# ppwwyyxx/speaker-recognition

Measured on AMD Instinct MI355X. Metric: frames/sec scored (MFCC+GMM), higher is better.
Workload: dtype f32

## Files before the change

### speaker-recognition_amd/csrc/mfcc_f64.hip

```cpp
#include "batch.hpp"
#include "mfcc.hpp"
#include "mfcc_dev.hpp"
#include "wave_ops.hpp"

#include <algorithm>

namespace sr {

static int &precision_flag() {
    static int v = 2;
    return v;
}
int mfcc_precision() { return precision_flag(); }
void mfcc_set_precision(int mode) { precision_flag() = mode == 0 ? 0 : 2; }

using d2 = double2;

__device__ __forceinline__ d2 mk(double x, double y) { return make_double2(x, y); }
__device__ __forceinline__ d2 dadd(d2 a, d2 b) { return mk(a.x + b.x, a.y + b.y); }
__device__ __forceinline__ d2 dsub(d2 a, d2 b) { return mk(a.x - b.x, a.y - b.y); }
__device__ __forceinline__ d2 dmul(d2 a, d2 b) { return mk(fma(-a.y, b.y, a.x * b.x), fma(a.y, b.x, a.x * b.y)); }
__device__ __forceinline__ d2 dmul_mi(d2 a) { return mk(a.y, -a.x); }
constexpr double DH = 0.70710678118654752440;
__device__ __forceinline__ d2 dmul_h_mh(d2 a) { return mk(DH * (a.x + a.y), DH * (a.y - a.x)); }
__device__ __forceinline__ d2 dmul_mh_mh(d2 a) { return mk(DH * (a.y - a.x), -DH * (a.x + a.y)); }

__device__ __forceinline__ d2 tw64(const d2 *t, int i, int nc) {
    d2 w = t[i & (nc - 1)];
    if (i & nc) w = mk(-w.x, -w.y);
    return w;
}

__device__ __forceinline__ void radix4d(d2 a, d2 b, d2 c, d2 d, d2 &y0, d2 &y1, d2 &y2, d2 &y3) {
    const d2 s0 = dadd(a, c), s1 = dsub(a, c), s2 = dadd(b, d), s3 = dmul_mi(dsub(b, d));
    y0 = dadd(s0, s2);
    y1 = dadd(s1, s3);
    y2 = dsub(s0, s2);
    y3 = dsub(s1, s3);
}

template <int NZ>
__device__ __forceinline__ void dft16d(d2 (&v)[16]) {
    constexpr double C1 = 0.92387953251128673848, S1 = 0.38268343236508978178;
    d2 u[4][4];
    if constexpr (NZ <= 4) {
#pragma unroll
        for (int q = 0; q < 4; q++)
#pragma unroll
            for (int r = 0; r < 4; r++) u[q][r] = v[q];
    } else {
#pragma unroll
        for (int q = 0; q < 4; q++) radix4d(v[q], v[4 + q], v[8 + q], v[12 + q], u[q][0], u[q][1], u[q][2], u[q][3]);
    }
    u[1][1] = dmul(u[1][1], mk(C1, -S1));
    u[1][2] = dmul_h_mh(u[1][2]);
    u[1][3] = dmul(u[1][3], mk(S1, -C1));
    u[2][1] = dmul_h_mh(u[2][1]);
    u[2][2] = dmul_mi(u[2][2]);
    u[2][3] = dmul_mh_mh(u[2][3]);
    u[3][1] = dmul(u[3][1], mk(S1, -C1));
    u[3][2] = dmul_mh_mh(u[3][2]);
    u[3][3] = dmul(u[3][3], mk(-C1, S1));
#pragma unroll
    for (int r = 0; r < 4; r++) radix4d(u[0][r], u[1][r], u[2][r], u[3][r], v[r], v[r + 4], v[r + 8], v[r + 12]);
}

template <int CTRL>
__device__ __forceinline__ float quad_f32(float x) {
    return __int_as_float(__builtin_amdgcn_update_dpp(0, __float_as_int(x), CTRL, 0xf, 0xf, true));
}
template <int CTRL>
__device__ __forceinline__ double quad_f64(double x) {
    union { double d; int i[2]; } a, b;
    a.d = x;
    b.i[0] = __builtin_amdgcn_update_dpp(0, a.i[0], CTRL, 0xf, 0xf, true);
    b.i[1] = __builtin_amdgcn_update_dpp(0, a.i[1], CTRL, 0xf, 0xf, true);
    return b.d;
}
constexpr int QUAD_XOR1 = 0xB1;
constexpr int QUAD_XOR2 = 0x4E;

__device__ constexpr double W32_COS[9] = {1.0, 0.98078528040323044913, 0.92387953251128675613, 0.83146961230254523708,
                                          0.70710678118654752440, 0.55557023301960222474, 0.38268343236508977173,
                                          0.19509032201612826785, 0.0};

__device__ __forceinline__ double ln_pos_f32(float e) {
    int ex;
    float m = frexpf(e, &ex);
    if (m < 0.70710678f) {
        m *= 2.0f;
        ex -= 1;
    }
    const double md = (double)m, den = md + 1.0;
    double r = (double)__builtin_amdgcn_rcpf((float)den);
    r = fma(r, fma(-den, r, 1.0), r);
    const double s = (md - 1.0) * r, s2 = s * s;
    double c15 = 1.0 / 15.0, c13 = 1.0 / 13.0, c11 = 1.0 / 11.0, c9 = 1.0 / 9.0, c7 = 1.0 / 7.0, c5 = 1.0 / 5.0, c3 = 1.0 / 3.0, ln2 = 0.69314718055994530942;
    asm volatile("" : "+s"(c15), "+s"(c13), "+s"(c11), "+s"(c9), "+s"(c7), "+s"(c5), "+s"(c3), "+s"(ln2));
    double p = c15;
    p = fma(p, s2, c13);
    p = fma(p, s2, c11);
    p = fma(p, s2, c9);
    p = fma(p, s2, c7);
    p = fma(p, s2, c5);
    p = fma(p, s2, c3);
    p = fma(p, s2, 1.0);
    return fma((double)ex, ln2, 2.0 * s * p);
}

constexpr int F64_WIN_BYTES = 4160;
constexpr int F64_WPB = 8;
constexpr int F64_U_ELEMS = 576;
constexpr int F64_PBUF_BYTE = F64_U_ELEMS * 16;
constexpr int F64_SE_BYTE = F64_PBUF_BYTE + 1100 * 4;
constexpr int F64_SLM_BYTE = F64_SE_BYTE + 272;
static_assert(F64_SLM_BYTE % 32 == 0 && F64_SLM_BYTE + 512 <= WAVE_SLAB_C * 16, "per-wave slab layout");

template <typename PcmT, int MP>
__global__ __launch_bounds__(64 * F64_WPB)
void mfcc_frames_fft2048_f64_kernel(const PcmT *__restrict__ pcm, const int64_t *__restrict__ sample_off,
                                    const int64_t *__restrict__ frame_off, int n_utt, int64_t n_frames,
                                    int64_t frames_per_wave, MfccDev p, MfccDev64 q, MelRuns mr, float *__restrict__ raw) {
    extern __shared__ __attribute__((aligned(32))) char smem[];
    constexpr int NC = 1024;
    float *s_melval = reinterpret_cast<float *>(smem);
    const int lane = threadIdx.x & 63;
    const int wave = threadIdx.x >> 6;
    double *s_win = reinterpret_cast<double *>(smem + (((size_t)mr.pad_floats * 4 + 31) & ~(size_t)31));
    char *slab_b = reinterpret_cast<char *>(s_win) + F64_WIN_BYTES + (size_t)wave * WAVE_SLAB_C * sizeof(d2);
    d2 *slab = reinterpret_cast<d2 *>(slab_b);
    float *pbuf = reinterpret_cast<float *>(slab_b + F64_PBUF_BYTE);
    float *s_e = reinterpret_cast<float *>(slab_b + F64_SE_BYTE);
    double *s_lm = reinterpret_cast<double *>(slab_b + F64_SLM_BYTE);

    for (int i = threadIdx.x; i < mr.pad_floats; i += 64 * F64_WPB) s_melval[i] = mr.pad_val[i];
    for (int i = threadIdx.x; i < F64_WIN_BYTES / 8; i += 64 * F64_WPB) s_win[i] = (i >= 1 && i <= p.frame_len) ? q.window[i - 1] : 0.0;
    __syncthreads();

    const d2 w1 = q.twiddle[2 * lane];
    const d2 wl = q.twiddle[lane];
    const int bb = lane & 15, gg = lane >> 4;
    const d2 w64_1 = q.twiddle[32 * bb];
    const int L = p.frame_len;
    const double lm_floor = q.mel_floor[lane];
    const int m_part = lane & 3, m_bl = lane >> 2;
    int m_c0[4];
#pragma unroll
    for (int ps = 0; ps < 4; ps++) m_c0[ps] = mr.col0[16 * ps + m_bl];

    const int64_t gwave = (int64_t)blockIdx.x * F64_WPB + wave;
    const int64_t f_begin = gwave * frames_per_wave;
    const int64_t f_end = f_begin + frames_per_wave < n_frames ? f_begin + frames_per_wave : n_frames;
    if (f_begin >= f_end) return;

    int utt = 0;
    {
        int lo = 0, hi = n_utt;
        while (hi - lo > 1) {
            const int mid = (lo + hi) >> 1;
            if (frame_off[mid] <= f_begin) lo = mid; else hi = mid;
        }
        utt = lo;
    }
    int64_t utt_f0 = frame_off[utt], utt_f1 = frame_off[utt + 1], utt_s0 = sample_off[utt];

    PcmT cm[4], c0[4], c1[4];
    auto fetch = [&](int64_t base) {
        const PcmT *fp = pcm + base;
#pragma unroll
        for (int n1 = 0; n1 < 4; n1++) {
            const int i0 = 2 * (64 * n1 + lane);
            c0[n1] = fp[min(i0, L - 1)];
            cm[n1] = fp[max(min(i0 - 1, L - 1), 0)];
            c1[n1] = fp[min(i0 + 1, L - 1)];
        }
    };
    fetch(utt_s0 + (f_begin - utt_f0) * p.frame_shift);

    for (int64_t frame = f_begin; frame < f_end; frame++) {
        d2 v[16];
#pragma unroll
        for (int n1 = 0; n1 < 4; n1++) {
            const int i0 = 2 * (64 * n1 + lane);
            const d2 wm0 = *reinterpret_cast<const d2 *>(s_win + i0);
            const double wp1 = s_win[i0 + 2];
            const double x0 = (double)c0[n1], xm = (double)cm[n1], x1 = (double)c1[n1];
            const double y0 = wm0.y * x0;
            const double re = fma(-(wm0.x * q.pre_emph), xm, y0);
            const double im = fma(-q.pre_emph, y0, wp1 * x1);
            v[n1] = mk(i0 < L ? re : 0.0, i0 + 1 < L ? im : 0.0);
        }
        if (frame + 1 < f_end) {
            int64_t nf = frame + 1;
            while (nf >= utt_f1) {
                utt++;
                utt_f0 = utt_f1;
                utt_f1 = frame_off[utt + 1];
                utt_s0 = sample_off[utt];
            }
            fetch(utt_s0 + (nf - utt_f0) * p.frame_shift);
        }
        dft16d<4>(v);
        {
            d2 cur = w1;
            v[1] = dmul(v[1], cur);
#pragma unroll
            for (int k1 = 2; k1 < 16; k1++) {
                cur = dmul(cur, w1);
                v[k1] = dmul(v[k1], cur);
            }
        }
        wave_sync();
#pragma unroll
        for (int k1 = 0; k1 < 16; k1++) slab[k1 * 68 + lane] = v[k1];
        wave_sync();
        {
            d2 w64_2 = dmul(w64_1, w64_1);
            asm volatile("" : "+v"(w64_2.x), "+v"(w64_2.y));
            const d2 w64_3 = dmul(w64_2, w64_1);
#pragma unroll
            for (int i = 0; i < 4; i++) {
                const d2 *rowp = slab + (4 * gg + i) * 68 + bb;
                radix4d(rowp[0], rowp[16], rowp[32], rowp[48], v[4 * i], v[4 * i + 1], v[4 * i + 2], v[4 * i + 3]);
                v[4 * i + 1] = dmul(v[4 * i + 1], w64_1);
                v[4 * i + 2] = dmul(v[4 * i + 2], w64_2);
                v[4 * i + 3] = dmul(v[4 * i + 3], w64_3);
            }
        }
        wave_sync();
#pragma unroll
        for (int i = 0; i < 4; i++)
#pragma unroll
            for (int c = 0; c < 4; c++) slab[((4 * gg + i) + 16 * c) * 17 + bb] = v[4 * i + c];
        wave_sync();
#pragma unroll
        for (int b = 0; b < 16; b++) v[b] = slab[lane * 17 + b];
        dft16d<16>(v);
        wave_sync();
#pragma unroll
        for (int d = 8; d < 16; d++) slab[(d - 8) * 64 + lane] = v[d];
        wave_sync();
        {
            const int src = (64 - lane) & 63;
            const int shift = lane == 0 ? 64 : 0;
#pragma unroll
            for (int d = 0; d < 8; d++) {
                const d2 zk = v[d];
                d2 zr = slab[(7 - d) * 64 + shift + src];
                if (d == 0 && lane == 0) zr = zk;
                const d2 e = mk(zk.x + zr.x, zk.y - zr.y);
                const d2 o = mk(zk.y + zr.y, zr.x - zk.x);
                d2 t;
                if (d == 0) t = dmul(wl, o);
                else if (d == 4) t = dmul(wl, dmul_h_mh(o));
                else t = dmul(wl, dmul(mk(W32_COS[d], -W32_COS[8 - d]), o));
                const d2 xp = dadd(e, t), xm = dsub(e, t);
                const int k = lane + 64 * d;
                pbuf[k] = (float)fma(xp.x, xp.x, xp.y * xp.y);
                pbuf[NC - k] = (float)fma(xm.x, xm.x, xm.y * xm.y);
            }
            if (lane == 0) pbuf[512] = (float)(4.0 * fma(v[8].x, v[8].x, v[8].y * v[8].y));
            pbuf[1025 + lane] = 0.f;
            if (lane < 11) pbuf[1089 + lane] = 0.f;
        }
        double dw[4][4];
        int dct_lane = lane;
        asm volatile("" : "+v"(dct_lane));
#pragma unroll
        for (int it = 0; it < 4; it++) {
            const double4 wv = reinterpret_cast<const double4 *>(q.dct_pad)[it * 64 + dct_lane];
            dw[it][0] = wv.x; dw[it][1] = wv.y; dw[it][2] = wv.z; dw[it][3] = wv.w;
        }
        wave_sync();
#pragma unroll
        for (int ps = 0; ps < 4; ps++) {
            const int len = mr.pass_len[ps];
            const float4 *mv4 = reinterpret_cast<const float4 *>(s_melval + mr.pass_base[ps]) + lane;
            int c0v = m_c0[ps];
            if constexpr (MP == 0) {
                int bl = 16 * ps + m_bl;
                asm volatile("" : "+v"(bl));
                c0v = mr.col0[bl];
            }
            const float4 *pp4 = reinterpret_cast<const float4 *>(pbuf + c0v) + m_part;
            float a0 = 0.f, a1 = 0.f, a2 = 0.f, a3 = 0.f;
            if constexpr (MP != 0) {
#pragma unroll
                for (int it = 0; it < mel_preset_steps(MP, ps); it++) {
                    const float4 wv = mv4[it * 64];
                    const float4 xv = pp4[it * 4];
                    a0 = fmaf(wv.x, xv.x, a0);
                    a1 = fmaf(wv.y, xv.y, a1);
                    a2 = fmaf(wv.z, xv.z, a2);
                    a3 = fmaf(wv.w, xv.w, a3);
                }
            } else {
                for (int it = 0; it < (len >> 4); it++) {
                    const float4 wv = mv4[it * 64];
                    const float4 xv = pp4[it * 4];
                    a0 = fmaf(wv.x, xv.x, a0);
                    a1 = fmaf(wv.y, xv.y, a1);
                    a2 = fmaf(wv.z, xv.z, a2);
                    a3 = fmaf(wv.w, xv.w, a3);
                }
            }
            float acc = (a0 + a1) + (a2 + a3);
            acc += quad_f32<QUAD_XOR1>(acc);
            acc += quad_f32<QUAD_XOR2>(acc);
            if (m_part == 0) s_e[16 * ps + m_bl] = acc;
        }
        wave_sync();
        {
            const float e = s_e[lane];
            s_lm[lane] = e > 0.f ? ln_pos_f32(e) : lm_floor;
        }
        wave_sync();
        {
            const int cidx = lane >> 2;
            const double4 *lp = reinterpret_cast<const double4 *>(s_lm) + m_part;
            double o0 = 0.0, o1 = 0.0;
#pragma unroll
            for (int it = 0; it < 4; it++) {
                const double4 lv = lp[it * 4];
                o0 = fma(dw[it][0], lv.x, o0);
                o1 = fma(dw[it][1], lv.y, o1);
                o0 = fma(dw[it][2], lv.z, o0);
                o1 = fma(dw[it][3], lv.w, o1);
            }
            double o = o0 + o1;
            o += quad_f64<QUAD_XOR1>(o);
            o += quad_f64<QUAD_XOR2>(o);
            if (m_part == 0 && cidx < p.n_ceps) raw[frame * p.n_ceps + cidx] = (float)o;
        }
    }
}

template <typename PcmT, int WPB>
__global__ __launch_bounds__(64 * WPB)
void mfcc_frames_f64_kernel(const PcmT *__restrict__ pcm, const int64_t *__restrict__ sample_off,
                            const int64_t *__restrict__ frame_off, int n_utt, int64_t n_frames,
                            MfccDev p, MfccDev64 q, float *__restrict__ raw ) {
    extern __shared__ __attribute__((aligned(16))) char smem[];
    const int nc = p.fft_size >> 1;
    d2 *s_tw = reinterpret_cast<d2 *>(smem);
    const int lane = threadIdx.x & 63;
    const int wave = threadIdx.x >> 6;
    d2 *buf_a = s_tw + nc + (size_t)wave * 2 * nc;
    d2 *buf_b = buf_a + nc;
    double *s_lm = reinterpret_cast<double *>(s_tw + nc + (size_t)WPB * 2 * nc) + wave * 64;

    for (int i = threadIdx.x; i < nc; i += 64 * WPB) s_tw[i] = q.twiddle[i];
    __syncthreads();

    const int64_t frames_per_iter = (int64_t)gridDim.x * WPB;
    const int64_t iters = (n_frames + frames_per_iter - 1) / frames_per_iter;
    for (int64_t it = 0; it < iters; it++) {
        const int64_t frame = (it * gridDim.x + blockIdx.x) * WPB + wave;
        const bool active = frame < n_frames;

        int64_t base = 0;
        if (active) {
            int lo = 0, hi = n_utt;
            while (hi - lo > 1) {
                const int mid = (lo + hi) >> 1;
                if (frame_off[mid] <= frame) lo = mid; else hi = mid;
            }
            base = sample_off[lo] + (frame - frame_off[lo]) * p.frame_shift;
        }

        if (active) {
            const int L = p.frame_len;
            for (int n = lane; n < nc; n += 64) {
                double re = 0.0, im = 0.0;
                const int i0 = 2 * n;
                if (i0 < L) {
                    const double c0 = (double)pcm[base + i0] * q.window[i0];
                    const double pm1 = i0 > 0 ? (double)pcm[base + i0 - 1] * q.window[i0 - 1] : 0.0;
                    re = i0 > 0 ? c0 - pm1 * q.pre_emph : c0;
                    if (i0 + 1 < L) {
                        const double c1 = (double)pcm[base + i0 + 1] * q.window[i0 + 1];
                        im = c1 - c0 * q.pre_emph;
                    }
                }
                buf_a[n] = mk(re, im);
            }
        }
        __syncthreads();

        d2 *in = buf_a, *out = buf_b;
        int ns = 1;
        for (; ns * 4 <= nc; ns *= 4) {
            if (active) {
                const int T = nc >> 2;
                const int tstep = p.fft_size / (4 * ns);
                for (int j = lane; j < T; j += 64) {
                    const int k = j & (ns - 1);
                    const int qq = k * tstep;
                    const d2 v0 = in[j];
                    const d2 v1 = dmul(in[j + T], tw64(s_tw, qq, nc));
                    const d2 v2 = dmul(in[j + 2 * T], tw64(s_tw, 2 * qq, nc));
                    const d2 v3 = dmul(in[j + 3 * T], tw64(s_tw, 3 * qq, nc));
                    d2 y0, y1, y2, y3;
                    radix4d(v0, v1, v2, v3, y0, y1, y2, y3);
                    const int j0 = ((j - k) << 2) + k;
                    out[j0] = y0;
                    out[j0 + ns] = y1;
                    out[j0 + 2 * ns] = y2;
                    out[j0 + 3 * ns] = y3;
                }
            }
            __syncthreads();
            d2 *t = in; in = out; out = t;
        }
        if (ns < nc) {
            if (active) {
                const int T = nc >> 1;
                for (int j = lane; j < T; j += 64) {
                    const d2 v0 = in[j];
                    const d2 v1 = dmul(in[j + T], tw64(s_tw, 2 * j, nc));
                    out[j] = dadd(v0, v1);
                    out[j + T] = dsub(v0, v1);
                }
            }
            __syncthreads();
            d2 *t = in; in = out; out = t;
        }

        double *pw = reinterpret_cast<double *>(out);
        if (active) {
            for (int k = lane; k <= nc; k += 64) {
                const d2 zk = in[k & (nc - 1)];
                const d2 zr = in[(nc - k) & (nc - 1)];
                const d2 e = mk(0.5 * (zk.x + zr.x), 0.5 * (zk.y - zr.y));
                const d2 o = mk(0.5 * (zk.y + zr.y), -0.5 * (zk.x - zr.x));
                const d2 x = dadd(e, dmul(tw64(s_tw, k, nc), o));
                const double pk = fma(x.x, x.x, x.y * x.y);
                pw[k] = pk < 1e-100 ? 1e-100 : pk;
            }
        }
        __syncthreads();

        if (active) {
            double mine = 0.0;
            for (int b = 0; b < p.n_filters; b++) {
                double acc = 0.0;
                const int e1 = p.mel_row[b + 1];
                for (int e = p.mel_row[b] + lane; e < e1; e += 64) acc = fma(q.mel_val[e], pw[p.mel_col[e]], acc);
                acc = wave_sum_f64(acc);
                if (lane == b) mine = acc > 0.0 ? log(acc) : q.mel_floor[b];
            }
            s_lm[lane] = mine;
        }
        __syncthreads();

        if (active && lane < p.n_ceps) {
            double acc = 0.0;
            const double *drow = q.dct + lane * p.n_filters;
            for (int b = 0; b < p.n_filters; b++) acc = fma(drow[b], s_lm[b], acc);
            raw[frame * p.n_ceps + lane] = (float)acc;
        }
        __syncthreads();
    }
}

void mfcc_launch_f64(SRMfcc &m, const MfccDev &dev, int pcm_kind, const void *pcm, const int64_t *d_pcm_off, const int64_t *d_raw_off,
                     int n_utt, int64_t n_frames, float *raw) {
    auto &tabs = device_tables(m);
    const MfccDev64 dev64 = device_tables_f64(m);
    const size_t mel_bytes = ((size_t)tabs.pad_floats * 4 + 31) & ~(size_t)31;
    const size_t lds_fast = mel_bytes + F64_WIN_BYTES + (size_t)F64_WPB * WAVE_SLAB_C * sizeof(d2);
    const bool fast = m.fft_size == 2048 && m.frame_len <= 512 && tabs.runs_contiguous && m.n_ceps <= 16 &&
                      lds_fast <= (size_t)160 * 1024 && !mfcc_force_generic();
    if (fast) {
        MelRuns mr;
        mr.col0 = tabs.mel_col0.p;
        mr.pad_val = tabs.mel_pad.p;
        mr.pad_floats = tabs.pad_floats;
        for (int ps = 0; ps < 4; ps++) {
            mr.pass_base[ps] = tabs.pass_base[ps];
            mr.pass_len[ps] = tabs.pass_len[ps];
        }
        const int64_t one_round = (int64_t)ctx().n_cu * F64_WPB;
        int64_t frames_per_wave = 1, best_cost = -1;
        for (int64_t r = 1; r <= 4; r++) {
            const int64_t fpw = std::max<int64_t>(1, (n_frames + r * one_round - 1) / (r * one_round));
            const int64_t waves = (n_frames + fpw - 1) / fpw;
            const int64_t cost = ((waves + one_round - 1) / one_round) * fpw;
            if (best_cost < 0 || cost < best_cost - best_cost / 50 || (cost <= best_cost + best_cost / 50 && fpw >= 32)) {
                best_cost = cost;
                frames_per_wave = fpw;
            }
        }
        const int64_t n_waves = (n_frames + frames_per_wave - 1) / frames_per_wave;
        const int grid = (int)((n_waves + F64_WPB - 1) / F64_WPB);
        int preset = 0;
        for (int pr = 1; pr <= 2 && !preset; pr++) {
            bool same = true;
            for (int ps = 0; ps < 4; ps++) same = same && tabs.pass_len[ps] == 16 * mel_preset_steps(pr, ps);
            if (same) preset = pr;
        }
#define SR_LAUNCH_F64(PT, MPV)                                                                              \
    do {                                                                                                     \
        auto kern = mfcc_frames_fft2048_f64_kernel<PT, MPV>;                                                 \
        SR_HIP(hipFuncSetAttribute(reinterpret_cast<const void *>(kern), hipFuncAttributeMaxDynamicSharedMemorySize, (int)lds_fast)); \
        hipLaunchKernelGGL(kern, dim3(grid), dim3(64 * F64_WPB), lds_fast, ctx().stream, static_cast<const PT *>(pcm), d_pcm_off,      \
                           d_raw_off, n_utt, n_frames, frames_per_wave, dev, dev64, mr, raw);                \
    } while (0)
#define SR_LAUNCH_F64_P(PT)                                                                                 \
    do {                                                                                                     \
        if (preset == 1) SR_LAUNCH_F64(PT, 1); else if (preset == 2) SR_LAUNCH_F64(PT, 2); else SR_LAUNCH_F64(PT, 0); \
    } while (0)
        if (pcm_kind == SRBatch::PCM16) SR_LAUNCH_F64_P(int16_t); else SR_LAUNCH_F64_P(float);
#undef SR_LAUNCH_F64_P
#undef SR_LAUNCH_F64
        return;
    }
    const int nc = m.fft_size / 2;
    auto lds_for = [&](int w) { return (size_t)nc * sizeof(d2) * (1 + 2 * w) + (size_t)w * 64 * sizeof(double); };
    const int wpb = lds_for(4) <= (size_t)160 * 1024 ? 4 : lds_for(2) <= (size_t)160 * 1024 ? 2 : 1;
    const size_t lds = lds_for(wpb);
    const int64_t blocks_needed = (n_frames + wpb - 1) / wpb;
    const int blocks_per_cu = std::max<int>(1, (int)(160 * 1024 / lds));
    const int grid = (int)std::min<int64_t>(blocks_needed, (int64_t)ctx().n_cu * std::min(blocks_per_cu, 8));
#define SR_LAUNCH_G64(PT, W)                                                                                \
    do {                                                                                                     \
        auto kern = mfcc_frames_f64_kernel<PT, W>;                                                           \
        SR_HIP(hipFuncSetAttribute(reinterpret_cast<const void *>(kern), hipFuncAttributeMaxDynamicSharedMemorySize, (int)lds)); \
        hipLaunchKernelGGL(kern, dim3(grid), dim3(64 * W), lds, ctx().stream, static_cast<const PT *>(pcm), d_pcm_off, d_raw_off, \
                           n_utt, n_frames, dev, dev64, raw);                                                \
    } while (0)
#define SR_LAUNCH_G64_W(PT)                                                                                 \
    do {                                                                                                     \
        if (wpb == 4) SR_LAUNCH_G64(PT, 4); else if (wpb == 2) SR_LAUNCH_G64(PT, 2); else SR_LAUNCH_G64(PT, 1); \
    } while (0)
    if (pcm_kind == SRBatch::PCM16) SR_LAUNCH_G64_W(int16_t); else SR_LAUNCH_G64_W(float);
#undef SR_LAUNCH_G64_W
#undef SR_LAUNCH_G64
}

}
```

Baseline: 37.11 million.

## Split each f64 MFCC frame across a two-wave team instead of one wave

The fp64 fast-path kernel now processes each frame with a 128-thread team of two waves, each doing half of the 1024-point complex FFT (radix-4 first stage with per-half twiddles, then two radix-8 stages). The untangle step and the mel filterbank sweep are divided between the two waves, and the DCT is left to wave 0. The mel weights are now read from global memory into registers instead of from an LDS copy, which shrinks LDS per block and allows more resident teams per CU. The aim is to cut per-wave register pressure and serial work per frame and raise occupancy, at the cost of block-level barriers and the DCT running on only one wave.

```diff
diff --git a/speaker-recognition_amd/csrc/mfcc_f64.hip b/speaker-recognition_amd/csrc/mfcc_f64.hip
--- a/speaker-recognition_amd/csrc/mfcc_f64.hip
+++ b/speaker-recognition_amd/csrc/mfcc_f64.hip
@@ -108,50 +108,87 @@
     return fma((double)ex, ln2, 2.0 * s * p);
 }
 
+__device__ __forceinline__ void dft8d(d2 (&x)[8]) {
+    d2 e0, e1, e2, e3, o0, o1, o2, o3;
+    radix4d(x[0], x[2], x[4], x[6], e0, e1, e2, e3);
+    radix4d(x[1], x[3], x[5], x[7], o0, o1, o2, o3);
+    o1 = dmul_h_mh(o1);
+    o2 = dmul_mi(o2);
+    o3 = dmul_mh_mh(o3);
+    x[0] = dadd(e0, o0);
+    x[1] = dadd(e1, o1);
+    x[2] = dadd(e2, o2);
+    x[3] = dadd(e3, o3);
+    x[4] = dsub(e0, o0);
+    x[5] = dsub(e1, o1);
+    x[6] = dsub(e2, o2);
+    x[7] = dsub(e3, o3);
+}
+
 constexpr int F64_WIN_BYTES = 4160;
-constexpr int F64_WPB = 8;
-constexpr int F64_U_ELEMS = 576;
-constexpr int F64_PBUF_BYTE = F64_U_ELEMS * 16;
-constexpr int F64_SE_BYTE = F64_PBUF_BYTE + 1100 * 4;
-constexpr int F64_SLM_BYTE = F64_SE_BYTE + 272;
-static_assert(F64_SLM_BYTE % 32 == 0 && F64_SLM_BYTE + 512 <= WAVE_SLAB_C * 16, "per-wave slab layout");
+constexpr int F64_TEAM_THREADS = 128;
+constexpr int F64_ROW = 72;
+constexpr int F64_REGION_C = 8 * F64_ROW;
+constexpr int F64_U_ROW = 72;
+constexpr int F64_PBUF_BYTE = (4 * F64_U_ROW + 1) * 16;
+constexpr int F64_SE_BYTE = 2 * F64_REGION_C * 16;
+constexpr int F64_SLM_BYTE = F64_SE_BYTE + 256;
+constexpr int F64_TEAM_BYTES = F64_SLM_BYTE + 512;
+constexpr int F64_TEAMS_PER_CU = 6;
+static_assert(F64_PBUF_BYTE + 1100 * 4 <= F64_REGION_C * 16, "the power spectrum must not reach wave 1's untangle rows");
+static_assert(F64_SLM_BYTE % 32 == 0 && F64_PBUF_BYTE % 16 == 0, "team slab layout");
+static_assert((size_t)F64_TEAMS_PER_CU * (F64_WIN_BYTES + F64_TEAM_BYTES) <= (size_t)160 * 1024, "teams per CU");
+
+#define SR_C1 0.92387953251128673848
+#define SR_S1 0.38268343236508978178
+#define SR_H 0.70710678118654752440
+__constant__ double F64_W16[2][2][6] = {{{1.0, 0.0, 1.0, 0.0, 1.0, 0.0}, {SR_C1, -SR_S1, SR_H, -SR_H, SR_S1, -SR_C1}},
+                                        {{SR_H, -SR_H, 0.0, -1.0, -SR_H, -SR_H}, {SR_S1, -SR_C1, -SR_H, -SR_H, -SR_C1, SR_S1}}};
+#undef SR_C1
+#undef SR_S1
+#undef SR_H
+
+template <int N>
+struct IntC { static constexpr int value = N; };
 
 template <typename PcmT, int MP>
-__global__ __launch_bounds__(64 * F64_WPB)
+__global__ __launch_bounds__(F64_TEAM_THREADS, 3)
 void mfcc_frames_fft2048_f64_kernel(const PcmT *__restrict__ pcm, const int64_t *__restrict__ sample_off,
                                     const int64_t *__restrict__ frame_off, int n_utt, int64_t n_frames,
-                                    int64_t frames_per_wave, MfccDev p, MfccDev64 q, MelRuns mr, float *__restrict__ raw) {
+                                    int64_t frames_per_team, MfccDev p, MfccDev64 q, MelRuns mr, float *__restrict__ raw) {
     extern __shared__ __attribute__((aligned(32))) char smem[];
     constexpr int NC = 1024;
-    float *s_melval = reinterpret_cast<float *>(smem);
+    const int64_t f_begin = (int64_t)blockIdx.x * frames_per_team;
+    const int64_t f_end = f_begin + frames_per_team < n_frames ? f_begin + frames_per_team : n_frames;
+    if (f_begin >= f_end) return;
+
     const int lane = threadIdx.x & 63;
-    const int wave = threadIdx.x >> 6;
-    double *s_win = reinterpret_cast<double *>(smem + (((size_t)mr.pad_floats * 4 + 31) & ~(size_t)31));
-    char *slab_b = reinterpret_cast<char *>(s_win) + F64_WIN_BYTES + (size_t)wave * WAVE_SLAB_C * sizeof(d2);
-    d2 *slab = reinterpret_cast<d2 *>(slab_b);
-    float *pbuf = reinterpret_cast<float *>(slab_b + F64_PBUF_BYTE);
-    float *s_e = reinterpret_cast<float *>(slab_b + F64_SE_BYTE);
-    double *s_lm = reinterpret_cast<double *>(slab_b + F64_SLM_BYTE);
-
-    for (int i = threadIdx.x; i < mr.pad_floats; i += 64 * F64_WPB) s_melval[i] = mr.pad_val[i];
-    for (int i = threadIdx.x; i < F64_WIN_BYTES / 8; i += 64 * F64_WPB) s_win[i] = (i >= 1 && i <= p.frame_len) ? q.window[i - 1] : 0.0;
+    const int hs = __builtin_amdgcn_readfirstlane(threadIdx.x >> 6);
+    double *s_win = reinterpret_cast<double *>(smem);
+    char *team_b = smem + F64_WIN_BYTES;
+    d2 *team = reinterpret_cast<d2 *>(team_b);
+    d2 *reg = team + hs * F64_REGION_C;
+    float *pbuf = reinterpret_cast<float *>(team_b + F64_PBUF_BYTE);
+    float *s_e = reinterpret_cast<float *>(team_b + F64_SE_BYTE);
+    double *s_lm = reinterpret_cast<double *>(team_b + F64_SLM_BYTE);
+
+    for (int i = threadIdx.x; i < F64_WIN_BYTES / 8; i += F64_TEAM_THREADS) s_win[i] = (i >= 1 && i <= p.frame_len) ? q.window[i - 1] : 0.0;
     __syncthreads();
 
-    const d2 w1 = q.twiddle[2 * lane];
-    const d2 wl = q.twiddle[lane];
-    const int bb = lane & 15, gg = lane >> 4;
-    const d2 w64_1 = q.twiddle[32 * bb];
+    const int lo3 = lane & 7, hi3 = lane >> 3;
+    const d2 tb0 = q.twiddle[2 * lane * (2 * hs)];
+    const d2 tb1 = q.twiddle[2 * lane * (2 * hs + 1)];
+    const d2 tw4 = q.twiddle[8 * lane];
+    const int k1 = 2 * hs + (lo3 & 1) + 4 * (lo3 >> 1);
+    const int m = k1 + 16 * hi3;
+    int u_src;
+    {
+        const int k1p = (16 - k1) & 15, cp = (k1 == 0 ? 8 : 7) - hi3;
+        u_src = ((k1p >> 1) & 1) * F64_REGION_C + cp * 9 + (k1p & 1) + 2 * (k1p >> 2);
+    }
     const int L = p.frame_len;
-    const double lm_floor = q.mel_floor[lane];
     const int m_part = lane & 3, m_bl = lane >> 2;
-    int m_c0[4];
-#pragma unroll
-    for (int ps = 0; ps < 4; ps++) m_c0[ps] = mr.col0[16 * ps + m_bl];
-
-    const int64_t gwave = (int64_t)blockIdx.x * F64_WPB + wave;
-    const int64_t f_begin = gwave * frames_per_wave;
-    const int64_t f_end = f_begin + frames_per_wave < n_frames ? f_begin + frames_per_wave : n_frames;
-    if (f_begin >= f_end) return;
+    const int m_c0a = MP ? mr.col0[16 * (hs ? 1 : 0) + m_bl] : 0, m_c0b = MP ? mr.col0[16 * (hs ? 2 : 3) + m_bl] : 0;
 
     int utt = 0;
     {
@@ -170,15 +207,66 @@
 #pragma unroll
         for (int n1 = 0; n1 < 4; n1++) {
             const int i0 = 2 * (64 * n1 + lane);
-            c0[n1] = fp[min(i0, L - 1)];
-            cm[n1] = fp[max(min(i0 - 1, L - 1), 0)];
-            c1[n1] = fp[min(i0 + 1, L - 1)];
+            c0[n1] = fp[(unsigned)min(i0, L - 1)];
+            cm[n1] = fp[(unsigned)max(min(i0 - 1, L - 1), 0)];
+            c1[n1] = fp[(unsigned)min(i0 + 1, L - 1)];
         }
     };
     fetch(utt_s0 + (f_begin - utt_f0) * p.frame_shift);
 
+    constexpr int NWA = MP ? mel_preset_steps(MP, 0) : 1, NWB = MP ? mel_preset_steps(MP, 3) : 1;
+    constexpr int NWC = MP ? mel_preset_steps(MP, 1) : 1, NWD = MP ? mel_preset_steps(MP, 2) : 1;
+    constexpr int NW = NWA + NWB > NWC + NWD ? NWA + NWB : NWC + NWD;
+    auto load_w = [&](auto psc, float4 *w) {
+        constexpr int ps = decltype(psc)::value;
+        int lane_f = lane;
+        asm volatile("" : "+v"(lane_f));
+        const float4 *mv4 = reinterpret_cast<const float4 *>(mr.pad_val + mr.pass_base[ps]) + lane_f;
+#pragma unroll
+        for (int it = 0; it < mel_preset_steps(MP, ps); it++) w[it] = mv4[it * 64];
+    };
+    auto sweep = [&](auto psc, int c0v, const float4 *w) {
+        constexpr int ps = decltype(psc)::value;
+        const float4 *pp4 = reinterpret_cast<const float4 *>(pbuf + c0v) + m_part;
+        float a0 = 0.f, a1 = 0.f, a2 = 0.f, a3 = 0.f;
+#pragma unroll
+        for (int it = 0; it < mel_preset_steps(MP, ps); it++) {
+            const float4 wv = w[it];
+            const float4 xv = pp4[it * 4];
+            a0 = fmaf(wv.x, xv.x, a0);
+            a1 = fmaf(wv.y, xv.y, a1);
+            a2 = fmaf(wv.z, xv.z, a2);
+            a3 = fmaf(wv.w, xv.w, a3);
+        }
+        float acc = (a0 + a1) + (a2 + a3);
+        acc += quad_f32<QUAD_XOR1>(acc);
+        acc += quad_f32<QUAD_XOR2>(acc);
+        if (m_part == 0) s_e[16 * ps + m_bl] = acc;
+    };
+    auto sweep_rt = [&](int ps) {
+        const int base = ps == 0 ? mr.pass_base[0] : ps == 1 ? mr.pass_base[1] : ps == 2 ? mr.pass_base[2] : mr.pass_base[3];
+        const int len = ps == 0 ? mr.pass_len[0] : ps == 1 ? mr.pass_len[1] : ps == 2 ? mr.pass_len[2] : mr.pass_len[3];
+        int bl = 16 * ps + m_bl;
+        asm volatile("" : "+v"(bl));
+        const float4 *mv4 = reinterpret_cast<const float4 *>(mr.pad_val + base) + (bl & 15) * 4 + m_part;
+        const float4 *pp4 = reinterpret_cast<const float4 *>(pbuf + mr.col0[bl]) + m_part;
+        float a0 = 0.f, a1 = 0.f, a2 = 0.f, a3 = 0.f;
+        for (int it = 0; it < (len >> 4); it++) {
+            const float4 wv = mv4[it * 64];
+            const float4 xv = pp4[it * 4];
+            a0 = fmaf(wv.x, xv.x, a0);
+            a1 = fmaf(wv.y, xv.y, a1);
+            a2 = fmaf(wv.z, xv.z, a2);
+            a3 = fmaf(wv.w, xv.w, a3);
+        }
+        float acc = (a0 + a1) + (a2 + a3);
+        acc += quad_f32<QUAD_XOR1>(acc);
+        acc += quad_f32<QUAD_XOR2>(acc);
+        if (m_part == 0) s_e[bl] = acc;
+    };
+
     for (int64_t frame = f_begin; frame < f_end; frame++) {
-        d2 v[16];
+        d2 u[4];
 #pragma unroll
         for (int n1 = 0; n1 < 4; n1++) {
             const int i0 = 2 * (64 * n1 + lane);
@@ -188,7 +276,7 @@
             const double y0 = wm0.y * x0;
             const double re = fma(-(wm0.x * q.pre_emph), xm, y0);
             const double im = fma(-q.pre_emph, y0, wp1 * x1);
-            v[n1] = mk(i0 < L ? re : 0.0, i0 + 1 < L ? im : 0.0);
+            u[n1] = mk(i0 < L ? re : 0.0, i0 + 1 < L ? im : 0.0);
         }
         if (frame + 1 < f_end) {
             int64_t nf = frame + 1;
@@ -200,122 +288,115 @@
             }
             fetch(utt_s0 + (nf - utt_f0) * p.frame_shift);
         }
-        dft16d<4>(v);
-        {
-            d2 cur = w1;
-            v[1] = dmul(v[1], cur);
-#pragma unroll
-            for (int k1 = 2; k1 < 16; k1++) {
-                cur = dmul(cur, w1);
-                v[k1] = dmul(v[k1], cur);
-            }
-        }
+        d2 v[8];
+        int hs_f = hs;
+        asm volatile("" : "+s"(hs_f));
+#pragma unroll
+        for (int r = 0; r < 2; r++) {
+            const double *wt = F64_W16[hs_f][r];
+            const d2 y1 = dmul(u[1], mk(wt[0], wt[1])), y2 = dmul(u[2], mk(wt[2], wt[3])), y3 = dmul(u[3], mk(wt[4], wt[5]));
+            radix4d(u[0], y1, y2, y3, v[r], v[r + 2], v[r + 4], v[r + 6]);
+            d2 cur = r == 0 ? tb0 : tb1;
+            v[r] = dmul(v[r], cur);
+#pragma unroll
+            for (int s = 1; s < 4; s++) {
+                cur = dmul(cur, tw4);
+                v[r + 2 * s] = dmul(v[r + 2 * s], cur);
+            }
+        }
+        int b_f = lo3;
+        asm volatile("" : "+v"(b_f));
+        const d2 w64_1 = q.twiddle[32 * b_f], w64_2 = q.twiddle[64 * b_f], w64_4 = q.twiddle[128 * b_f];
         wave_sync();
 #pragma unroll
-        for (int k1 = 0; k1 < 16; k1++) slab[k1 * 68 + lane] = v[k1];
+        for (int j = 0; j < 8; j++) reg[j * F64_ROW + lane] = v[j];
         wave_sync();
         {
-            d2 w64_2 = dmul(w64_1, w64_1);
-            asm volatile("" : "+v"(w64_2.x), "+v"(w64_2.y));
-            const d2 w64_3 = dmul(w64_2, w64_1);
-#pragma unroll
-            for (int i = 0; i < 4; i++) {
-                const d2 *rowp = slab + (4 * gg + i) * 68 + bb;
-                radix4d(rowp[0], rowp[16], rowp[32], rowp[48], v[4 * i], v[4 * i + 1], v[4 * i + 2], v[4 * i + 3]);
-                v[4 * i + 1] = dmul(v[4 * i + 1], w64_1);
-                v[4 * i + 2] = dmul(v[4 * i + 2], w64_2);
-                v[4 * i + 3] = dmul(v[4 * i + 3], w64_3);
-            }
+            const d2 *rowp = reg + hi3 * F64_ROW + lo3;
+#pragma unroll
+            for (int a = 0; a < 8; a++) v[a] = rowp[8 * a];
+            dft8d(v);
+            const d2 w64_3 = dmul(w64_2, w64_1), w64_6 = dmul(w64_4, w64_2), w64_5 = dmul(w64_4, w64_1);
+            v[1] = dmul(v[1], w64_1);
+            v[2] = dmul(v[2], w64_2);
+            v[3] = dmul(v[3], w64_3);
+            v[4] = dmul(v[4], w64_4);
+            v[5] = dmul(v[5], w64_5);
+            v[6] = dmul(v[6], w64_6);
+            v[7] = dmul(v[7], dmul(w64_6, w64_1));
         }
         wave_sync();
 #pragma unroll
-        for (int i = 0; i < 4; i++)
-#pragma unroll
-            for (int c = 0; c < 4; c++) slab[((4 * gg + i) + 16 * c) * 17 + bb] = v[4 * i + c];
-        wave_sync();
-#pragma unroll
-        for (int b = 0; b < 16; b++) v[b] = slab[lane * 17 + b];
-        dft16d<16>(v);
-        wave_sync();
-#pragma unroll
-        for (int d = 8; d < 16; d++) slab[(d - 8) * 64 + lane] = v[d];
+        for (int c = 0; c < 8; c++) reg[c * F64_ROW + hi3 * 9 + lo3] = v[c];
         wave_sync();
         {
-            const int src = (64 - lane) & 63;
-            const int shift = lane == 0 ? 64 : 0;
-#pragma unroll
-            for (int d = 0; d < 8; d++) {
+            const d2 *colp = reg + hi3 * F64_ROW + lo3 * 9;
+#pragma unroll
+            for (int b = 0; b < 8; b++) v[b] = colp[b];
+        }
+        dft8d(v);
+        wave_sync();
+#pragma unroll
+        for (int d = 4; d < 8; d++) reg[(d - 4) * F64_U_ROW + hi3 * 9 + lo3] = v[d];
+        int m_f = m;
+        asm volatile("" : "+v"(m_f));
+        const d2 wl = q.twiddle[m_f];
+        __syncthreads();
+        {
+#pragma unroll
+            for (int d = 0; d < 4; d++) {
                 const d2 zk = v[d];
-                d2 zr = slab[(7 - d) * 64 + shift + src];
-                if (d == 0 && lane == 0) zr = zk;
+                d2 zr = team[(3 - d) * F64_U_ROW + u_src];
+                if (d == 0 && m == 0) zr = zk;
                 const d2 e = mk(zk.x + zr.x, zk.y - zr.y);
                 const d2 o = mk(zk.y + zr.y, zr.x - zk.x);
                 d2 t;
                 if (d == 0) t = dmul(wl, o);
-                else if (d == 4) t = dmul(wl, dmul_h_mh(o));
-                else t = dmul(wl, dmul(mk(W32_COS[d], -W32_COS[8 - d]), o));
+                else if (d == 2) t = dmul(wl, dmul_h_mh(o));
+                else t = dmul(wl, dmul(mk(W32_COS[2 * d], -W32_COS[8 - 2 * d]), o));
                 const d2 xp = dadd(e, t), xm = dsub(e, t);
-                const int k = lane + 64 * d;
+                const int k = m + 128 * d;
                 pbuf[k] = (float)fma(xp.x, xp.x, xp.y * xp.y);
                 pbuf[NC - k] = (float)fma(xm.x, xm.x, xm.y * xm.y);
             }
-            if (lane == 0) pbuf[512] = (float)(4.0 * fma(v[8].x, v[8].x, v[8].y * v[8].y));
-            pbuf[1025 + lane] = 0.f;
-            if (lane < 11) pbuf[1089 + lane] = 0.f;
-        }
-        double dw[4][4];
-        int dct_lane = lane;
-        asm volatile("" : "+v"(dct_lane));
-#pragma unroll
-        for (int it = 0; it < 4; it++) {
-            const double4 wv = reinterpret_cast<const double4 *>(q.dct_pad)[it * 64 + dct_lane];
-            dw[it][0] = wv.x; dw[it][1] = wv.y; dw[it][2] = wv.z; dw[it][3] = wv.w;
-        }
-        wave_sync();
-#pragma unroll
-        for (int ps = 0; ps < 4; ps++) {
-            const int len = mr.pass_len[ps];
-            const float4 *mv4 = reinterpret_cast<const float4 *>(s_melval + mr.pass_base[ps]) + lane;
-            int c0v = m_c0[ps];
-            if constexpr (MP == 0) {
-                int bl = 16 * ps + m_bl;
-                asm volatile("" : "+v"(bl));
-                c0v = mr.col0[bl];
-            }
-            const float4 *pp4 = reinterpret_cast<const float4 *>(pbuf + c0v) + m_part;
-            float a0 = 0.f, a1 = 0.f, a2 = 0.f, a3 = 0.f;
-            if constexpr (MP != 0) {
-#pragma unroll
-                for (int it = 0; it < mel_preset_steps(MP, ps); it++) {
-                    const float4 wv = mv4[it * 64];
-                    const float4 xv = pp4[it * 4];
-                    a0 = fmaf(wv.x, xv.x, a0);
-                    a1 = fmaf(wv.y, xv.y, a1);
-                    a2 = fmaf(wv.z, xv.z, a2);
-                    a3 = fmaf(wv.w, xv.w, a3);
-                }
+            if (m == 0) pbuf[512] = (float)(4.0 * fma(v[4].x, v[4].x, v[4].y * v[4].y));
+            if (threadIdx.x < 75) pbuf[1025 + threadIdx.x] = 0.f;
+        }
+        float4 mw[NW];
+        if constexpr (MP != 0) {
+            if (hs == 0) {
+                load_w(IntC<0>{}, mw);
+                load_w(IntC<3>{}, mw + NWA);
             } else {
-                for (int it = 0; it < (len >> 4); it++) {
-                    const float4 wv = mv4[it * 64];
-                    const float4 xv = pp4[it * 4];
-                    a0 = fmaf(wv.x, xv.x, a0);
-                    a1 = fmaf(wv.y, xv.y, a1);
-                    a2 = fmaf(wv.z, xv.z, a2);
-                    a3 = fmaf(wv.w, xv.w, a3);
-                }
-            }
-            float acc = (a0 + a1) + (a2 + a3);
-            acc += quad_f32<QUAD_XOR1>(acc);
-            acc += quad_f32<QUAD_XOR2>(acc);
-            if (m_part == 0) s_e[16 * ps + m_bl] = acc;
-        }
-        wave_sync();
-        {
-            const float e = s_e[lane];
-            s_lm[lane] = e > 0.f ? ln_pos_f32(e) : lm_floor;
-        }
-        wave_sync();
-        {
+                load_w(IntC<1>{}, mw);
+                load_w(IntC<2>{}, mw + NWC);
+            }
+        }
+        __syncthreads();
+        if constexpr (MP == 0) {
+            for (int i = 0; i < 2; i++) sweep_rt(hs ? 1 + i : 3 * i);
+        } else if (hs == 0) {
+            sweep(IntC<0>{}, m_c0a, mw);
+            sweep(IntC<3>{}, m_c0b, mw + NWA);
+        } else {
+            sweep(IntC<1>{}, m_c0a, mw);
+            sweep(IntC<2>{}, m_c0b, mw + NWC);
+        }
+        __syncthreads();
+        if (hs == 0) {
+            double dw[4][4];
+            int dct_lane = lane;
+            asm volatile("" : "+v"(dct_lane));
+#pragma unroll
+            for (int it = 0; it < 4; it++) {
+                const double4 wv = reinterpret_cast<const double4 *>(q.dct_pad)[it * 64 + dct_lane];
+                dw[it][0] = wv.x; dw[it][1] = wv.y; dw[it][2] = wv.z; dw[it][3] = wv.w;
+            }
+            {
+                const float e = s_e[lane];
+                s_lm[lane] = e > 0.f ? ln_pos_f32(e) : q.mel_floor[dct_lane];
+            }
+            wave_sync();
             const int cidx = lane >> 2;
             const double4 *lp = reinterpret_cast<const double4 *>(s_lm) + m_part;
             double o0 = 0.0, o1 = 0.0;
@@ -467,10 +548,8 @@
                      int n_utt, int64_t n_frames, float *raw) {
     auto &tabs = device_tables(m);
     const MfccDev64 dev64 = device_tables_f64(m);
-    const size_t mel_bytes = ((size_t)tabs.pad_floats * 4 + 31) & ~(size_t)31;
-    const size_t lds_fast = mel_bytes + F64_WIN_BYTES + (size_t)F64_WPB * WAVE_SLAB_C * sizeof(d2);
-    const bool fast = m.fft_size == 2048 && m.frame_len <= 512 && tabs.runs_contiguous && m.n_ceps <= 16 &&
-                      lds_fast <= (size_t)160 * 1024 && !mfcc_force_generic();
+    const size_t lds_fast = F64_WIN_BYTES + F64_TEAM_BYTES;
+    const bool fast = m.fft_size == 2048 && m.frame_len <= 512 && tabs.runs_contiguous && m.n_ceps <= 16 && !mfcc_force_generic();
     if (fast) {
         MelRuns mr;
         mr.col0 = tabs.mel_col0.p;
@@ -480,19 +559,18 @@
             mr.pass_base[ps] = tabs.pass_base[ps];
             mr.pass_len[ps] = tabs.pass_len[ps];
         }
-        const int64_t one_round = (int64_t)ctx().n_cu * F64_WPB;
-        int64_t frames_per_wave = 1, best_cost = -1;
+        const int64_t one_round = (int64_t)ctx().n_cu * F64_TEAMS_PER_CU;
+        int64_t frames_per_team = 1, best_cost = -1;
         for (int64_t r = 1; r <= 4; r++) {
-            const int64_t fpw = std::max<int64_t>(1, (n_frames + r * one_round - 1) / (r * one_round));
-            const int64_t waves = (n_frames + fpw - 1) / fpw;
-            const int64_t cost = ((waves + one_round - 1) / one_round) * fpw;
-            if (best_cost < 0 || cost < best_cost - best_cost / 50 || (cost <= best_cost + best_cost / 50 && fpw >= 32)) {
+            const int64_t fpt = std::max<int64_t>(1, (n_frames + r * one_round - 1) / (r * one_round));
+            const int64_t teams = (n_frames + fpt - 1) / fpt;
+            const int64_t cost = ((teams + one_round - 1) / one_round) * fpt;
+            if (best_cost < 0 || cost < best_cost - best_cost / 50 || (cost <= best_cost + best_cost / 50 && fpt >= 32)) {
                 best_cost = cost;
-                frames_per_wave = fpw;
-            }
-        }
-        const int64_t n_waves = (n_frames + frames_per_wave - 1) / frames_per_wave;
-        const int grid = (int)((n_waves + F64_WPB - 1) / F64_WPB);
+                frames_per_team = fpt;
+            }
+        }
+        const int grid = (int)((n_frames + frames_per_team - 1) / frames_per_team);
         int preset = 0;
         for (int pr = 1; pr <= 2 && !preset; pr++) {
             bool same = true;
@@ -503,8 +581,8 @@
     do {                                                                                                     \
         auto kern = mfcc_frames_fft2048_f64_kernel<PT, MPV>;                                                 \
         SR_HIP(hipFuncSetAttribute(reinterpret_cast<const void *>(kern), hipFuncAttributeMaxDynamicSharedMemorySize, (int)lds_fast)); \
-        hipLaunchKernelGGL(kern, dim3(grid), dim3(64 * F64_WPB), lds_fast, ctx().stream, static_cast<const PT *>(pcm), d_pcm_off,      \
-                           d_raw_off, n_utt, n_frames, frames_per_wave, dev, dev64, mr, raw);                \
+        hipLaunchKernelGGL(kern, dim3(grid), dim3(F64_TEAM_THREADS), lds_fast, ctx().stream, static_cast<const PT *>(pcm), d_pcm_off, \
+                           d_raw_off, n_utt, n_frames, frames_per_team, dev, dev64, mr, raw);                \
     } while (0)
 #define SR_LAUNCH_F64_P(PT)                                                                                 \
     do {                                                                                                     \
```

Result: slower. 34.54 million (-6.9%).
